# scroll-tech/scroll-prover

Measured on AMD Instinct MI355X. Metric: BN254 MSM G1-adds/sec at k=26, higher is better.
Workload: dtype u32 (9x29-bit limbs of 254-bit Montgomery integers; v_mad_u64_u32); 1 GPU; BN254 G1 Pippenger MSM, 2^26 uniform random scalars x synthetic SRS points, inputs resident in HBM; point-range shards over 1 GPU(s), RCCL all-gather of 96-B partials; log_n=26, window_bits=22, windows=12, parallelism=point-range x1, one rank per GPU, srs_window_tables=True

## Files before the change

### scroll-prover_amd/csrc/lib_msm.hip

```cpp
#define ZK_FRSCAN_DEVICE_ONLY 1
#include "msm.hpp"
#define ZK_G2_DEVICE_ONLY 1
#include "msm_g2.hpp"
#include "msm_seg.hpp"
#include "lib_common.hpp"

namespace mi355 {

static_assert(sizeof(fe_t) == 32 && sizeof(g1_affine_t) == 64 && sizeof(g1_jac_t) == 96, "ABI element sizes");
static_assert(sizeof(g1_xyzz_t) == 128 && sizeof(g1_xyzz29_t) == 144, "device record sizes (workspace layout, 16-byte vector accesses)");

int msm_tu_init_device() {
  HIPCHK(hipFuncSetAttribute((const void *)k_sort_l1_scatter_split<24>, hipFuncAttributeMaxDynamicSharedMemorySize, 160 * 1024));
  HIPCHK(hipFuncSetAttribute((const void *)k_sort_l1_scatter_split<16>, hipFuncAttributeMaxDynamicSharedMemorySize, 160 * 1024));
  HIPCHK(hipFuncSetAttribute((const void *)k_sort_l1_scatter_split<8>, hipFuncAttributeMaxDynamicSharedMemorySize, 160 * 1024));
  HIPCHK(hipFuncSetAttribute((const void *)k_sort_l2_scatter_split<16>, hipFuncAttributeMaxDynamicSharedMemorySize, 160 * 1024));
  HIPCHK(hipFuncSetAttribute((const void *)k_sort_l2_scatter_split<8>, hipFuncAttributeMaxDynamicSharedMemorySize, 160 * 1024));
  return MI355_OK;
}

double msm_cost(uint64_t n, int c, bool shared) { const double W = (MSM_SCALAR_BITS + c - 1) / c, nb = (double)(1ull << (c - 1)); return 1.18 * W * (double)n + 8.2 * nb * (shared ? 1.0 : W) + (shared ? 0.0 : 3.0e7); }

int choose_c(uint64_t n) {
  if (t_opts.force_c) return t_opts.force_c;
// ... 80 lines not shown
  int32_t *lv_ids; rec_t *lv_recs;
  CHK(ws.get("segfix_ids", cap * 4, lv_ids)); CHK(ws.get("segfix_recs", cap * sizeof(rec_t), lv_recs));
  const int32_t *cur_ids = part_id; const rec_t *cur_recs = part; size_t used = 0;
  while (N > 64) {
    const uint32_t waves = ceil_div(N, 64);
    hipLaunchKernelGGL(k_msm_segfix<G>, dim3(ceil_div(N, 256)), dim3(256), 0, s, cur_ids, cur_recs, N, buckets, lv_ids + used, lv_recs + used, 0);
    cur_ids = lv_ids + used; cur_recs = lv_recs + used; used += (size_t)2 * waves; N = 2 * waves;
  }
  hipLaunchKernelGGL(k_msm_segfix<G>, dim3(1), dim3(64), 0, s, cur_ids, cur_recs, N, buckets, (int32_t *)nullptr, (rec_t *)nullptr, 1);
  return MI355_OK;
}

template <class G> int msm_reduce_tail(const MsmShape &sh, uint32_t M, const typename G::rec_t *buckets, typename G::out_t *out_dev, bool normalise, hipStream_t s, const Roles &ws) {
  using rec_t = typename G::rec_t;
  const uint32_t nb = 1u << (sh.c - 1), wpp = sh.shared ? 1 : sh.W, sets = M * wpp;
  uint32_t chunk = 64; while (chunk > nb) chunk >>= 1;
  while (chunk > g.reduce_min_chunk && (uint64_t)(nb / chunk) * sets < g.reduce_chains) chunk >>= 1;
  const uint32_t chunks_per_set = nb / chunk, nchunks = chunks_per_set * sets;
  rec_t *chunk_out, *tree_a, *tree_b, *window_sums;
  CHK(ws.get("chunk_out", (size_t)nchunks * sizeof(rec_t), chunk_out));
  { const size_t lvl = (size_t)ceil_div(chunks_per_set, 64 * TREE_PER_THREAD) * sets + 1;
    CHK(ws.get("tree_a", lvl * sizeof(rec_t), tree_a)); CHK(ws.get("tree_b", lvl * sizeof(rec_t), tree_b)); }
  CHK(ws.get("window_sums", (size_t)sets * sizeof(rec_t), window_sums));
  with_lanes<G>(nchunks <= g.tail_coop_max && (g.tail_coop_mask & 2u), [&](auto q) {
    constexpr int Q = decltype(q)::value;
    hipLaunchKernelGGL((k_msm_bucket_reduce<G, Q>), dim3(ceil_div((uint64_t)nchunks * Q, 128)), dim3(128), 0, s, buckets, chunk_out, nb, sets, chunk);
  });
  const rec_t *cur = chunk_out; uint32_t cnt = chunks_per_set; rec_t *bufs[2] = {tree_a, tree_b}; int which = 0;
  while (true) {
    const bool coop = G::QUAD && (uint64_t)cnt * sets <= g.tail_coop_max && (g.tail_coop_mask & 4u);
    const uint32_t outn = ceil_div(cnt, (coop ? 64u : 256u) * TREE_PER_THREAD);
    rec_t *dst = outn == 1 ? window_sums : bufs[which];
    with_lanes<G>(coop, [&](auto q) { hipLaunchKernelGGL((k_msm_tree_sum<G, decltype(q)::value>), dim3(outn, sets), dim3(256), 0, s, cur, cnt, dst, outn); });
    if (outn == 1) break;
    cur = dst; cnt = outn; which ^= 1;
  }
  with_lanes<G>(g.tail_coop_max && (g.tail_coop_mask & 8u), [&](auto q) {
    hipLaunchKernelGGL((k_msm_final<G, decltype(q)::value>), dim3(M), dim3(64), 0, s, (const rec_t *)window_sums, wpp, sh.shared ? 0u : sh.c, out_dev, normalise ? 1 : 0);
  });
  HIPCHK(hipGetLastError());
  return MI355_OK;
}

int msm_sort_stage(const PolyPtrs &inl, const fe_t *const *polys_dev, uint32_t M, uint64_t n, const MsmShape &sh, const MsmPlan &P, uint32_t *offsets, uint32_t *sorted,
                   hipStream_t s, bool g2 = false) {
  const bool shared = sh.shared;
  const uint64_t emax = sh.emax;
  const uint32_t nbuckets = (uint32_t)sh.nbuckets;
  SortPlan S; S.n = P.n; S.windows = M * P.windows; S.wpp = P.windows; S.nb = P.nb;
  S.fb = sh.fb; S.cb_bits = sh.cb_bits;
  S.shared = shared ? 1 : 0; S.nshift = log2_ceil(n);
  S.regions = sh.regions;
  S.t1 = g.sort_t1;
  if (g.sort_split == 1 && S.t1 == 16384 && (1u << S.cb_bits) <= 1024 && emax >= (1ull << 24)) S.t1 = 24576;
  S.t2 = g.sort_t2 ? g.sort_t2 : (emax >= (1ull << 27) && S.fb <= 11 ? 16384 : 8192);
  const uint32_t tiles1 = ceil_div(n, S.t1), l2_tiles_max = ceil_div(emax, S.t2) + S.regions + 8;
  const uint32_t vwindows = M * P.windows;

  uint32_t *enc, *hist, *cursor, *scan_sums, *coarse_hist, *coarse_off, *coarse_cursor, *tile_start;
  CHK(ws_get("msm.digits", emax * 4, (void **)&enc));
  uint32_t *pairs_lo = nullptr; uint16_t *pairs_hi = nullptr;
  CHK(ws_get("msm.pairs_lo", emax * 4 + 64, (void **)&pairs_lo)); CHK(ws_get("msm.pairs_hi", emax * 2 + 64, (void **)&pairs_hi));
  CHK(ws_get("msm.hist", ((size_t)nbuckets + 1) * 4, (void **)&hist));
  CHK(ws_get("msm.cursor", ((size_t)nbuckets + 1) * 4, (void **)&cursor));
  CHK(ws_get("msm.coarse_hist", ((size_t)S.regions + 1) * 4, (void **)&coarse_hist));
  CHK(ws_get("msm.coarse_off", ((size_t)S.regions + 1) * 4, (void **)&coarse_off));
  CHK(ws_get("msm.coarse_cursor", ((size_t)S.regions + 1) * 4, (void **)&coarse_cursor));
  CHK(ws_get("msm.tile_start", ((size_t)S.regions + 1) * 4, (void **)&tile_start));
  const uint32_t scan_n = nbuckets + 1, scan_blocks = ceil_div(scan_n, SCAN_BLOCK * SCAN_ITEMS);
  const uint32_t cscan_n = S.regions + 1, cscan_blocks = ceil_div(cscan_n, SCAN_BLOCK * SCAN_ITEMS);
  CHK(ws_get("msm.scan_sums", (size_t)(scan_blocks + cscan_blocks) * 4, (void **)&scan_sums));
  const int grid_stream = g.prop.multiProcessorCount * 8;
  {
    Scope sc(g2 ? "msm_g2_digits" : "msm_digits", s);
    HIPCHK(hipMemsetAsync(coarse_hist, 0, ((size_t)S.regions + 1) * 4, s));
    const dim3 dgrid(grid_stream / M > 0 ? grid_stream / M : 1, M);
    if (g2) hipLaunchKernelGGL(k_msm_digits<false>, dgrid, dim3(256), (size_t)S.regions * 4, s, inl, polys_dev, enc, P, coarse_hist, S.fb, S.cb_bits, S.shared);
    else hipLaunchKernelGGL(k_msm_digits<true>, dgrid, dim3(256), (size_t)S.regions * 4, s, inl, polys_dev, enc, P, coarse_hist, S.fb, S.cb_bits, S.shared);
  }
  {
    Scope sc(g2 ? "msm_g2_sort" : "msm_sort", s);
    HIPCHK(hipMemsetAsync(hist, 0, ((size_t)nbuckets + 1) * 4, s));
    hipLaunchKernelGGL(k_scan_partial, dim3(cscan_blocks), dim3(SCAN_BLOCK), 0, s, coarse_hist, scan_sums + scan_blocks, cscan_n);
    hipLaunchKernelGGL(k_scan_block_sums, dim3(1), dim3(SCAN_BLOCK), 0, s, scan_sums + scan_blocks, cscan_blocks);
    hipLaunchKernelGGL(k_scan_final, dim3(cscan_blocks), dim3(SCAN_BLOCK), 0, s, coarse_hist, scan_sums + scan_blocks, coarse_off, coarse_cursor, cscan_n);
    {
      Scope s1(g2 ? "g2_sort_l1" : "sort_l1", s);
      const uint32_t CBp = ((1u << S.cb_bits) + 1) & ~1u;
      const size_t lds1 = (size_t)(3 * CBp + 32 + SORT_SPLIT_TMAX) * 4 + (size_t)S.t1 * 6;
      if (S.t1 == 24576) hipLaunchKernelGGL(k_sort_l1_scatter_split<24>, dim3(tiles1 * vwindows), dim3(1024), lds1, s, enc, coarse_cursor, pairs_lo, pairs_hi, S);
      else if (S.t1 == 16384) hipLaunchKernelGGL(k_sort_l1_scatter_split<16>, dim3(tiles1 * vwindows), dim3(1024), lds1, s, enc, coarse_cursor, pairs_lo, pairs_hi, S);
      else hipLaunchKernelGGL(k_sort_l1_scatter_split<8>, dim3(tiles1 * vwindows), dim3(1024), lds1, s, enc, coarse_cursor, pairs_lo, pairs_hi, S);
    }
    hipLaunchKernelGGL(k_sort_tile_prefix, dim3(1), dim3(SCAN_BLOCK), 0, s, coarse_off, tile_start, S);
    { Scope s2(g2 ? "g2_sort_hist" : "sort_hist", s);
    hipLaunchKernelGGL(k_sort_l2_hist_split, dim3(l2_tiles_max), dim3(256), 0, s, (const uint16_t *)pairs_hi, coarse_off, tile_start, hist, S); }
    hipLaunchKernelGGL(k_scan_partial, dim3(scan_blocks), dim3(SCAN_BLOCK), 0, s, hist, scan_sums, scan_n);
    hipLaunchKernelGGL(k_scan_block_sums, dim3(1), dim3(SCAN_BLOCK), 0, s, scan_sums, scan_blocks);
    hipLaunchKernelGGL(k_scan_final, dim3(scan_blocks), dim3(SCAN_BLOCK), 0, s, hist, scan_sums, offsets, cursor, scan_n);
    {
      Scope s3(g2 ? "g2_sort_l2" : "sort_l2", s);
      const size_t lds2 = (size_t)(3 * (1u << S.fb) + 32) * 4 + (size_t)S.t2 * 6;
      if (S.t2 == 8192) hipLaunchKernelGGL(k_sort_l2_scatter_split<8>, dim3(l2_tiles_max), dim3(1024), lds2, s, (const uint32_t *)pairs_lo, (const uint16_t *)pairs_hi, coarse_off, tile_start, cursor, sorted, S);
      else hipLaunchKernelGGL(k_sort_l2_scatter_split<16>, dim3(l2_tiles_max), dim3(1024), lds2, s, (const uint32_t *)pairs_lo, (const uint16_t *)pairs_hi, coarse_off, tile_start, cursor, sorted, S);
    }
  }
  return MI355_OK;
}

struct MsmStreams { hipStream_t a, b, c; };

int msm_enqueue(const g1_affine_t *bases, const PolyPtrs &inl, const fe_t *const *polys_dev, uint32_t M, uint64_t n, g1_jac_t *out_dev, const PreTable *pre, MsmSlot &slot,
                const MsmStreams &st, bool normalise, const MsmShape *forced = nullptr, uint32_t set_index = 0, uint32_t set_count = 1, bool skip_tail = false) {
  const bool piped = st.a != st.b;
  const Roles ws{G1Ops::ROLE, slot.id ? "#" + std::to_string(slot.id) : std::string()};
  MsmShape sh; CHK(msm_shape(n, M, pre, sh, forced));
  const bool shared = sh.shared;
  if (shared) bases = pre->table;
  const uint64_t emax = sh.emax;
  const AccPlan ap = msm_acc_plan(emax);
  const MsmPlan P = msm_plan(sh, n, M, ap.seg);
  const bool segfix = g.fixup_mode == 1 || (g.fixup_mode == 2 && (uint32_t)sh.nbuckets >= (1u << 19) && (uint64_t)P.seg * sh.nbuckets >= emax);
  const uint32_t seg_arg = msm_seg_arg(P.seg, segfix ? g.seg_fill_segfix : g.seg_fill);
  const uint32_t nbuckets = (uint32_t)sh.nbuckets;
  const uint32_t acc_blocks = ap.blocks, tn = ap.tn;
  uint32_t *offsets, *sorted;
  g1_xyzz29_t *buckets, *part; int32_t *part_id;
  CHK(ws.get("offsets", ((size_t)nbuckets + 1) * 4, offsets));
  CHK(ws.get("sorted", emax * 4, sorted));
  CHK(ws.get("buckets", (size_t)nbuckets * set_count * sizeof(g1_xyzz29_t), buckets));
  buckets += (size_t)nbuckets * set_index;
  CHK(ws.get("part", (size_t)tn * 2 * sizeof(g1_xyzz29_t), part));
  CHK(ws.get("part_id", (size_t)tn * 2 * 4, part_id));
  const uint32_t big_cap = tn / g.fixup_serial_max + 2;
  uint32_t *big_list; CHK(ws.get("big_list", ((size_t)big_cap * 3 + 1) * 4, big_list));
  uint32_t *big_count = big_list + (size_t)big_cap * 3;
  const uint32_t huge_cap = tn / FIXUP_HUGE_MIN + 2;
  uint32_t *huge_list, *huge_count; g1_xyzz29_t *huge_part;
  CHK(ws.get("huge_list", ((size_t)huge_cap * 3 + 1) * 4, huge_list)); huge_count = huge_list + (size_t)huge_cap * 3;
  CHK(ws.get("huge_part", (size_t)huge_cap * FIXUP_SLICES * sizeof(g1_xyzz29_t), huge_part));

  {
    hipStream_t s = st.a;
    if (piped && slot.used) { HIPCHK(hipStreamWaitEvent(s, slot.acc_done, 0)); HIPCHK(hipStreamWaitEvent(s, slot.red_done, 0)); }
    CHK(msm_sort_stage(inl, polys_dev, M, n, sh, P, offsets, sorted, s));
    if (piped) { HIPCHK(hipEventRecord(slot.sorted, s)); HIPCHK(hipStreamWaitEvent(st.b, slot.sorted, 0)); }
  }
  {
    hipStream_t s = st.b;
    if (piped && slot.used) HIPCHK(hipStreamWaitEvent(s, slot.red_done, 0));
    {
      Scope sc("msm_accumulate", s);
      HIPCHK(hipMemsetAsync(buckets, 0, (size_t)nbuckets * sizeof(g1_xyzz29_t), s));
      hipLaunchKernelGGL(k_msm_accumulate, dim3(acc_blocks), dim3(256), 0, s, bases, sorted, offsets, nbuckets, buckets, part, part_id, seg_arg, log2_ceil(n), shared ? pre->row_stride : (uint64_t)0);
    }
    if (piped) { HIPCHK(hipEventRecord(slot.acc_done, s)); HIPCHK(hipStreamWaitEvent(st.c, slot.acc_done, 0)); }
  }
  {
    hipStream_t s = st.c;
    Scope sc("msm_reduce", s);
    HIPCHK(hipMemsetAsync(big_count, 0, 4, s));
    HIPCHK(hipMemsetAsync(huge_count, 0, 4, s));
    if (segfix) CHK(msm_segfix_levels<G1Ops>(part_id, part, tn, buckets, s, ws));
    else {
      auto fixup = [&](auto kernel, uint64_t threads) {
        hipLaunchKernelGGL(kernel, dim3(ceil_div(threads, 256)), dim3(256), 0, s, offsets, nbuckets, buckets, part, part_id, seg_arg, tn, big_list, big_count, big_cap, huge_list, huge_count, huge_cap, g.fixup_serial_max, g.fixup_huge_min);
      };
      if ((uint64_t)nbuckets * 4 <= g.tail_coop_max && (g.tail_coop_mask & 1u)) fixup(k_msm_fixup<4, 4>, (uint64_t)nbuckets * 16);
      else if (nbuckets <= (1u << g.fixup_lanes_max_log)) fixup(k_msm_fixup<4, 1>, (uint64_t)nbuckets * 4);
      else fixup(k_msm_fixup<1, 1>, nbuckets);
      hipLaunchKernelGGL(k_msm_fixup_big, dim3(big_cap), dim3(256), 0, s, buckets, part, part_id, big_list, big_count);
      hipLaunchKernelGGL(k_msm_fixup_huge, dim3(huge_cap * FIXUP_SLICES), dim3(256), 0, s, part, part_id, huge_list, huge_count, huge_part, huge_cap);
      hipLaunchKernelGGL(k_msm_fixup_huge_fold, dim3(huge_cap), dim3(64), 0, s, buckets, huge_list, huge_count, (const g1_xyzz29_t *)huge_part);
    }
    if (!skip_tail) CHK(msm_reduce_tail<G1Ops>(sh, M, buckets, out_dev, normalise, s, ws));
  }
  if (piped) HIPCHK(hipEventRecord(slot.red_done, st.c));
  slot.used = true;
  HIPCHK(hipGetLastError());
  g.last_c = (int)P.c; g.last_w = (int)P.windows; g.last_entries += emax; g.last_shared = shared;
  return MI355_OK;
}

uint32_t msm_chunks_for(uint32_t M, uint64_t n) {
  if (g.msm_chunks <= 1 || M != 1 || n < (1ull << g.msm_chunk_min_log)) return 1;
  uint32_t k = g.msm_chunks;
  while (k > 1 && n / k < ((1ull << g.msm_chunk_min_log) >> 2)) k--;
  return k;
}

int msm_deliver(CallTrace &tr, const g1_jac_t *out_dev, uint32_t M, void *out_host, void *out_dev_user, hipStream_t s, const char *what, uint32_t count) {
  if (out_dev_user) {
    HIPCHK(hipMemcpyAsync(out_dev_user, out_dev, (size_t)M * sizeof(g1_jac_t), hipMemcpyDeviceToDevice, s));
    if (g.profiling) resolve_spans();
    tr.done(" (device result)");
    return MI355_OK;
  }
  HIPCHK(hipMemcpyAsync(out_host, out_dev, (size_t)M * sizeof(g1_jac_t), hipMemcpyDeviceToHost, s));
  HIPCHK(hipStreamSynchronize(s));
  resolve_spans();
  { char buf[64]; snprintf(buf, sizeof buf, " %s=%u c=%d W=%d", what, count, g.last_c, g.last_w); tr.done(buf); }
  return MI355_OK;
}

int msm_batch_impl(const g1_affine_t *bases, const fe_t *const *polys_host, uint32_t M, uint64_t n, void *out_host, const PreTable *pre, void *out_dev_user = nullptr, bool accumulate_plan = false) {
  if (M == 0) return MI355_OK;
  if (n == 0) {
    if (out_dev_user) { HIPCHK(hipMemsetAsync(out_dev_user, 0, (size_t)M * sizeof(g1_jac_t), g.stream)); return MI355_OK; }
    memset(out_host, 0, (size_t)M * sizeof(g1_jac_t)); return MI355_OK;
  }
  if (n >= (1ull << 31)) return fail(MI355_EBADARG, "msm: n must be < 2^31");
  if (M > 1 && msm_batch_must_split<G1Ops>(n, M, pre)) {
    const uint32_t h = M / 2;
    CHK(msm_batch_impl(bases, polys_host, h, n, out_host, pre, out_dev_user, accumulate_plan));
    return msm_batch_impl(bases, polys_host + h, M - h, n, out_host ? (char *)out_host + (size_t)h * sizeof(g1_jac_t) : nullptr, pre,
                          out_dev_user ? (char *)out_dev_user + (size_t)h * sizeof(g1_jac_t) : nullptr, true);
  }
  const uint32_t K = msm_chunks_for(M, n);
  if (!accumulate_plan) { g.last_entries = 0; g.last_host_slices = 1; }
  CallTrace tr("msm_g1", (uint64_t)M * n, 96.0);
  g1_jac_t *out_dev; const fe_t **polys_dev = nullptr;
  CHK(ws_get("msm.out", (size_t)(K + 1) * M * sizeof(g1_jac_t), (void **)&out_dev));
  hipStream_t s = g.stream;
  Scope total("msm_total", s);
  PolyPtrs inl{};
  if (K == 1) {
    CHK(msm_stage_polys(polys_host, M, Roles{G1Ops::ROLE, ""}, s, inl, polys_dev));
    MsmStreams st{s, s, s};
    CHK(msm_enqueue(bases, inl, polys_dev, M, n, out_dev, pre, g.msm_slot[0], st, t_opts.normalise));
  } else {
    std::vector<uint64_t> lo(K + 1);
    for (uint32_t k = 0; k <= K; k++) lo[k] = n * k / K;
    HIPCHK(hipEventRecord(g.ev_fork, s));
    HIPCHK(hipStreamWaitEvent(g.aux_stream[0], g.ev_fork, 0)); HIPCHK(hipStreamWaitEvent(g.aux_stream[1], g.ev_fork, 0));
    MsmStreams st{g.aux_stream[0], s, g.aux_stream[1]};
    for (uint32_t k = 0; k < K; k++) {
      PreTable pk; const PreTable *pp = pre_advance(pre, lo[k], pk);
      inl.p[0] = polys_host[0] + lo[k];
      CHK(msm_enqueue(bases + lo[k], inl, nullptr, M, lo[k + 1] - lo[k], out_dev + (size_t)(k + 1) * M, pp, g.msm_slot[k & 1], st, false));
    }
    HIPCHK(hipStreamWaitEvent(s, g.msm_slot[0].red_done, 0)); HIPCHK(hipStreamWaitEvent(s, g.msm_slot[1].red_done, 0));
    HIPCHK(hipEventRecord(g.ev_fork, st.a)); HIPCHK(hipStreamWaitEvent(s, g.ev_fork, 0));
    hipLaunchKernelGGL(k_g1_sum_strided, dim3(M), dim3(64), 0, s, out_dev + M, K, M, out_dev, t_opts.normalise ? 1 : 0);
  }
  HIPCHK(hipGetLastError());
  total.close();
  g.msm_slot[0].used = g.msm_slot[1].used = false;
  g.last_chunks = (int)K;
  return msm_deliver(tr, out_dev, M, out_host, out_dev_user, s, "batch", M);
}

int msm_host_single(const g1_affine_t *bases, const fe_t *const *polys_host, uint32_t M, uint64_t n, void *out_host, const PreTable *pre, void *out_dev_user = nullptr) {
  fe_t *sc; CHK(ws_get("io.scalars", (size_t)M * n * sizeof(fe_t), (void **)&sc));
  hipStream_t s = g.stream;
  std::vector<uint64_t> cut;
  if (M == 1 && n >= (1ull << g.host_slice_min_log) && g.host_chunks > 1) {
    double w = 1.0, tot = 0; std::vector<double> ws;
    const double first = 1.0 / 16.0;
    for (double rem = 1.0; rem > 1e-9 && ws.size() + 1 < g.host_chunks;) { const double take = std::min(rem, first * w); ws.push_back(take); rem -= take; w *= 1.7; tot += take; }
    if (tot < 1.0 - 1e-9) ws.push_back(1.0 - tot);
    cut.push_back(0); double acc = 0;
    const uint64_t align = n >= (1ull << 20) ? ~1023ull : ~0ull;
    for (size_t i = 0; i + 1 < ws.size(); i++) { acc += ws[i]; const uint64_t c = std::min<uint64_t>(n, (uint64_t)(acc * (double)n) & align); if (c > cut.back() && c < n) cut.push_back(c); }
    cut.push_back(n);
  }
  uint32_t K = cut.empty() ? 1 : (uint32_t)cut.size() - 1;
  uint64_t biggest = 0; for (uint32_t k = 0; k < K && !cut.empty(); k++) biggest = std::max(biggest, cut[k + 1] - cut[k]);
  MsmShape shape;
  if (K > 1 && (msm_shape(biggest, 1, pre, shape) != MI355_OK || shape.nbuckets * K * sizeof(g1_xyzz29_t) > (8ull << 30))) K = 1;
  if (K <= 1) {
    std::vector<const fe_t *> ptrs(M);
    for (uint32_t m = 0; m < M; m++) { ptrs[m] = sc + (size_t)m * n; HIPCHK(hipMemcpyAsync(sc + (size_t)m * n, polys_host[m], n * sizeof(fe_t), hipMemcpyHostToDevice, s)); }
    return msm_batch_impl(bases, ptrs.data(), M, n, out_host, pre, out_dev_user);
  }
  g.last_entries = 0;
  CallTrace tr("msm_g1_host", n, 96.0);
  g1_jac_t *out_dev; CHK(ws_get("msm.out", 2 * sizeof(g1_jac_t), (void **)&out_dev));
  Scope total("msm_total", s);
  HIPCHK(hipEventRecord(g.ev_fork, s)); HIPCHK(hipStreamWaitEvent(g.copy_stream, g.ev_fork, 0));
  PolyPtrs inl{};
  MsmStreams st{s, s, s};
  for (uint32_t k = 0; k < K; k++) {
    const uint64_t lo = cut[k], hi = cut[k + 1];
    HIPCHK(hipMemcpyAsync(sc + lo, polys_host[0] + lo, (hi - lo) * sizeof(fe_t), hipMemcpyHostToDevice, g.copy_stream));
    HIPCHK(hipEventRecord(g.ev_copy[k & 3], g.copy_stream));
    HIPCHK(hipStreamWaitEvent(s, g.ev_copy[k & 3], 0));
    PreTable pk; const PreTable *pp = pre_advance(pre, lo, pk);
    inl.p[0] = sc + lo;
    CHK(msm_enqueue(bases + lo, inl, nullptr, 1, hi - lo, out_dev, pp, g.msm_slot[0], st, t_opts.normalise, &shape, k, K, true));
  }
  g.msm_slot[0].used = false;
  g1_xyzz29_t *buckets; CHK(ws_get("msm.buckets", (size_t)shape.nbuckets * K * sizeof(g1_xyzz29_t), (void **)&buckets));
  {
    Scope sc2("msm_reduce", s);
    hipLaunchKernelGGL(k_msm_bucket_fold, dim3(ceil_div(shape.nbuckets, 256)), dim3(256), 0, s, buckets, (uint32_t)shape.nbuckets, K);
    CHK(msm_reduce_tail<G1Ops>(shape, 1, buckets, out_dev, t_opts.normalise, s, Roles{G1Ops::ROLE, ""}));
  }
  total.close();
  g.last_chunks = (int)K; g.last_host_slices = (int)K;
  return msm_deliver(tr, out_dev, 1, out_host, out_dev_user, s, "host slices", K);
}

static int msm_g2_impl(const g2_affine_t *bases, const fe_t *const *polys, uint32_t M, uint64_t n, void *out_host, bool accumulate_plan = false) {
  if (M == 0) return MI355_OK;
  if (n == 0) { memset(out_host, 0, (size_t)M * sizeof(g2_affine_t)); return MI355_OK; }
  if (n >= (1ull << 31)) return fail(MI355_EBADARG, "msm_g2: n must be < 2^31");
// ... 618 lines not shown
```

### scroll-prover_amd/csrc/msm.hpp

```cpp
#pragma once
#include "fp_asm.hpp"
#include "g1_29.hpp"
#include "frscan.hpp"

namespace zk {

#if defined(__HIPCC__)

struct MsmPlan {
  uint32_t n;
  uint32_t c;
  uint32_t windows;
  uint32_t nb;
  uint32_t seg;
  uint32_t batch;
};

__device__ __forceinline__ g1_affine_t load_affine(const g1_affine_t *p) {
  g1_affine_t r; r.x = g_load(&p->x); r.y = g_load(&p->y); return r;
}
__device__ __forceinline__ g1_affine_t load_affine_nt(const g1_affine_t *p) {
  const uint32_t *q = reinterpret_cast<const uint32_t *>(p); g1_affine_t r;
#pragma unroll
  for (int i = 0; i < 8; i++) { r.x.l[i] = __builtin_nontemporal_load(q + i); r.y.l[i] = __builtin_nontemporal_load(q + 8 + i); }
// ... 213 lines not shown
__device__ __forceinline__ void tile_bin_publish(uint32_t *gbase, const uint32_t *lstart, const uint32_t (&gb)[4], uint32_t nbins) {
  const uint32_t bpt = (nbins + 1023) >> 10, b0 = threadIdx.x * bpt;
  for (uint32_t k = 0; k < 4; k++) if (k < bpt && b0 + k < nbins) gbase[b0 + k] = gb[k] - lstart[b0 + k];
}
template <int EPT> __global__ void __launch_bounds__(1024) k_sort_l1_scatter_split(const uint32_t *__restrict__ enc, uint32_t *__restrict__ coarse_cursor, uint32_t *__restrict__ pairs_lo,
                                                                                    uint16_t *__restrict__ pairs_hi, SortPlan S) {
  extern __shared__ uint32_t sm[];
  const uint32_t CB = 1u << S.cb_bits, CBp = (CB + 1) & ~1u, fmask = (1u << S.fb) - 1;
  const uint32_t spare = 16u - S.fb, rmask = (1u << spare) - 1, tcount = (CB + rmask) >> spare;
  uint32_t *h = sm, *lstart = sm + CBp, *gbase = sm + 2 * CBp, *scratch32 = sm + 3 * CBp, *T = sm + 3 * CBp + 32;
  uint32_t *stage_lo = T + SORT_SPLIT_TMAX;
  uint16_t *stage_hi = reinterpret_cast<uint16_t *>(stage_lo + 1024 * EPT);
  const uint32_t tiles1 = (S.n + S.t1 - 1) / S.t1;
  const uint32_t w = blockIdx.x / tiles1, j = blockIdx.x - w * tiles1;
  for (uint32_t b = threadIdx.x; b < CB; b += 1024) h[b] = 0;
  __syncthreads();
  const uint32_t i0 = j * S.t1, i1 = min(S.n, i0 + S.t1);
  const uint32_t *plane = enc + (uint64_t)w * S.n;
  uint32_t e[EPT], rank[EPT];
#pragma unroll
  for (int k = 0; k < EPT; k++) {
    const uint32_t i = i0 + k * 1024 + threadIdx.x;
    e[k] = i < i1 ? plane[i] : 0;
  }
  asm volatile("s_waitcnt vmcnt(0)" ::: "memory");
#pragma unroll
  for (int k = 0; k < EPT; k++) if (e[k]) rank[k] = atomicAdd(&h[((e[k] & 0x7fffffffu) - 1) >> S.fb], 1u);
  __syncthreads();
  const uint32_t m_poly = w / S.wpp, w_in = w - m_poly * S.wpp;
  uint32_t gb[4];
  const uint32_t total = tile_bin_offsets(h, lstart, gb, CB, coarse_cursor + (S.shared ? m_poly * CB : w * CB), scratch32);
  const uint32_t idx_base = S.shared ? w_in << S.nshift : 0;
  __syncthreads();
  for (uint32_t k = threadIdx.x; k < tcount; k += 1024) T[k] = lstart[k << spare];
#pragma unroll
  for (int k = 0; k < EPT; k++) if (e[k]) {
    const uint32_t bucket = (e[k] & 0x7fffffffu) - 1, i = i0 + k * 1024 + threadIdx.x, bin = bucket >> S.fb, pos = lstart[bin] + rank[k];
    stage_lo[pos] = (idx_base + i) | (e[k] & 0x80000000u);
    stage_hi[pos] = (uint16_t)((bucket & fmask) | ((bin & rmask) << S.fb));
  }
  tile_bin_publish(gbase, lstart, gb, CB);
  __syncthreads();
  uint32_t k = 0;
  for (uint32_t sidx = threadIdx.x; sidx < total; sidx += 1024) {
    const uint32_t key = stage_hi[sidx];
    while (k + 1 < tcount && T[k + 1] <= sidx) k++;
    const uint32_t bin = (k << spare) | (key >> S.fb), pos = gbase[bin] + sidx;
    pairs_lo[pos] = stage_lo[sidx]; pairs_hi[pos] = (uint16_t)(key & fmask);
  }
}
__global__ void __launch_bounds__(SCAN_BLOCK) k_sort_tile_prefix(const uint32_t *__restrict__ coarse_off, uint32_t *__restrict__ tile_start, SortPlan S) {
  __shared__ uint32_t lds[32];
  __shared__ uint32_t running;
  if (threadIdx.x == 0) running = 0;
  __syncthreads();
  for (uint32_t base = 0; base < S.regions; base += SCAN_BLOCK) {
    const uint32_t r = base + threadIdx.x;
    const uint32_t v = r < S.regions ? (coarse_off[r + 1] - coarse_off[r] + S.t2 - 1) / S.t2 : 0;
    uint32_t total; const uint32_t ex = block_exclusive_scan(v, lds, total);
    const uint32_t run = running;
    if (r < S.regions) tile_start[r] = run + ex;
    __syncthreads();
    if (threadIdx.x == 0) running = run + total;
    __syncthreads();
  }
  if (threadIdx.x == 0) tile_start[S.regions] = running;
}
__device__ __forceinline__ bool sort_l2_tile(const uint32_t *__restrict__ coarse_off, const uint32_t *__restrict__ tile_start, const SortPlan &S, uint32_t &region, uint32_t &s, uint32_t &e) {
  const uint32_t total = tile_start[S.regions], per_xcd = (total + 7) >> 3, q = blockIdx.x >> 3;
  const uint32_t tile = (blockIdx.x & 7) * per_xcd + q;
  if (q >= per_xcd || tile >= total) return false;
  uint32_t lo = 0, hi = S.regions;
  while (hi - lo > 1) { const uint32_t mid = (lo + hi) >> 1; if (tile_start[mid] <= tile) lo = mid; else hi = mid; }
  region = lo;
  s = coarse_off[lo] + (tile - tile_start[lo]) * S.t2;
  e = min(coarse_off[lo + 1], s + S.t2);
  return true;
}
__global__ void __launch_bounds__(256) k_sort_l2_hist_split(const uint16_t *__restrict__ pairs_hi, const uint32_t *__restrict__ coarse_off, const uint32_t *__restrict__ tile_start,
                                                            uint32_t *__restrict__ hist, SortPlan S) {
  __shared__ uint32_t h[SORT_MAX_BINS];
  uint32_t region, s, e;
  if (!sort_l2_tile(coarse_off, tile_start, S, region, s, e)) return;
  const uint32_t FB = 1u << S.fb;
  for (uint32_t b = threadIdx.x; b < FB; b += blockDim.x) h[b] = 0;
  __syncthreads();
  const uint32_t a0 = min(e, (s + 7u) & ~7u), a1 = a0 + ((e - a0) & ~7u);
  for (uint32_t p = s + threadIdx.x; p < a0; p += blockDim.x) atomicAdd(&h[pairs_hi[p]], 1u);
  for (uint32_t q = a0 + 8u * threadIdx.x; q < a1; q += 8u * blockDim.x) {
    const uint4 v = *reinterpret_cast<const uint4 *>(pairs_hi + q);
    atomicAdd(&h[v.x & 0xffffu], 1u); atomicAdd(&h[v.x >> 16], 1u); atomicAdd(&h[v.y & 0xffffu], 1u); atomicAdd(&h[v.y >> 16], 1u);
    atomicAdd(&h[v.z & 0xffffu], 1u); atomicAdd(&h[v.z >> 16], 1u); atomicAdd(&h[v.w & 0xffffu], 1u); atomicAdd(&h[v.w >> 16], 1u);
  }
  for (uint32_t p = a1 + threadIdx.x; p < e; p += blockDim.x) atomicAdd(&h[pairs_hi[p]], 1u);
  __syncthreads();
  for (uint32_t b = threadIdx.x; b < FB; b += blockDim.x) if (h[b]) atomicAdd(&hist[(region << S.fb) + b], h[b]);
}
template <int EPT> __global__ void __launch_bounds__(1024) k_sort_l2_scatter_split(const uint32_t *__restrict__ pairs_lo, const uint16_t *__restrict__ pairs_hi, const uint32_t *__restrict__ coarse_off,
                                                                                    const uint32_t *__restrict__ tile_start, uint32_t *__restrict__ cursor, uint32_t *__restrict__ sorted, SortPlan S) {
  extern __shared__ uint32_t sm[];
  const uint32_t FB = 1u << S.fb;
  uint32_t *h = sm, *lstart = sm + FB, *gbase = sm + 2 * FB, *scratch32 = sm + 3 * FB, *stage = sm + 3 * FB + 32;
  uint32_t region, s, e;
  if (!sort_l2_tile(coarse_off, tile_start, S, region, s, e)) return;
  for (uint32_t b = threadIdx.x; b < FB; b += 1024) h[b] = 0;
  __syncthreads();
  uint32_t idx[EPT], fine[EPT], rank[EPT];
#pragma unroll
  for (int k = 0; k < EPT; k++) {
    const uint32_t p = s + k * 1024 + threadIdx.x;
    fine[k] = 0xffffffffu;
    if (p < e) { idx[k] = pairs_lo[p]; fine[k] = pairs_hi[p]; }
  }
  asm volatile("s_waitcnt vmcnt(0)" ::: "memory");
#pragma unroll
  for (int k = 0; k < EPT; k++) if (fine[k] != 0xffffffffu) rank[k] = atomicAdd(&h[fine[k]], 1u);
  __syncthreads();
  uint32_t gb[4];
  const uint32_t total = tile_bin_offsets(h, lstart, gb, FB, cursor + (region << S.fb), scratch32);
  __syncthreads();
  uint16_t *stage_bin = reinterpret_cast<uint16_t *>(stage + 1024 * EPT);
#pragma unroll
  for (int k = 0; k < EPT; k++) if (fine[k] != 0xffffffffu) { const uint32_t pos = lstart[fine[k]] + rank[k]; stage[pos] = idx[k]; stage_bin[pos] = (uint16_t)fine[k]; }
  tile_bin_publish(gbase, lstart, gb, FB);
  __syncthreads();
  for (uint32_t sidx = threadIdx.x; sidx < total; sidx += 1024) {
    const uint32_t b = stage_bin[sidx];
    sorted[gbase[b] + sidx] = stage[sidx];
  }
}

__device__ __forceinline__ uint32_t msm_seg_eff(uint32_t total, uint32_t threads, uint32_t seg_arg) {
  const uint32_t seg_max = seg_arg & 0x1fffu, seg_min = (seg_arg >> 13) & 0x1fffu, fill_pct = (seg_arg >> 26) * 2;
  const uint64_t target = ((uint64_t)threads * (fill_pct > 100u ? 100u : fill_pct) + 99) / 100;
  uint32_t sg = (uint32_t)(((uint64_t)total + target - 1) / (target ? target : 1));
  sg = sg < seg_min ? seg_min : sg;
  return sg > seg_max ? seg_max : sg;
}
template <class G, class B> __device__ __forceinline__ void msm_segment_walk(const B &bases, const uint32_t *__restrict__ sorted, const uint32_t *__restrict__ offsets, uint32_t nbuckets,
                                                                              typename G::rec_t *__restrict__ bucket_sums, typename G::rec_t *__restrict__ part, int32_t *__restrict__ part_id, uint32_t seg_arg,
                                                                              uint32_t t, uint32_t threads) {
  const uint32_t total = offsets[nbuckets];
  const uint32_t seg = msm_seg_eff(total, threads, seg_arg);
  const uint64_t start64 = (uint64_t)t * seg;
  if (start64 >= total) { part_id[2 * t] = -1; part_id[2 * t + 1] = -1; return; }
  const uint32_t start = (uint32_t)start64, end = (uint32_t)min((uint64_t)total, start64 + seg);
  uint32_t lo = 0, hi = nbuckets;
  while (hi - lo > 1) { const uint32_t mid = (lo + hi) >> 1; if (offsets[mid] <= start) lo = mid; else hi = mid; }
  uint32_t b = lo, b_start = offsets[b], b_end = offsets[b + 1];
  int32_t id_first = -1, id_last = -1;
  typename G::rec_t acc = G::identity();
  uint32_t ent = sorted[start];
  uint32_t ent_next = start + 1 < end ? sorted[start + 1] : 0;
  typename B::base_t p = bases.load(ent);
  for (uint32_t pos = start; pos < end; pos++) {
    typename B::base_t p_next = p;
    if (pos + 1 < end) { ent_next = sorted[pos + 1]; p_next = bases.load(ent_next); }
    if (pos >= b_end) {
      if (b_start >= start) G::store(&bucket_sums[b], acc);
      else { G::store(&part[2 * (uint64_t)t], acc); id_first = (int32_t)b; }
      acc = G::identity();
      b++; b_start = b_end; b_end = offsets[b + 1];
      if (pos >= b_end) {
        uint32_t l2 = b, h2 = nbuckets;
        while (h2 - l2 > 1) { const uint32_t mid = (l2 + h2) >> 1; if (offsets[mid] <= pos) l2 = mid; else h2 = mid; }
        b = l2; b_start = offsets[b]; b_end = offsets[b + 1];
      }
    }
    bases.madd(acc, p, (ent >> 31) != 0);
    ent = ent_next; p = p_next;
  }
  if (b_start >= start && b_end <= end) G::store(&bucket_sums[b], acc);
  else if (b_start < start) { G::store(&part[2 * (uint64_t)t], acc); id_first = (int32_t)b; }
  else { G::store(&part[2 * (uint64_t)t + 1], acc); id_last = (int32_t)b; }
  part_id[2 * t] = id_first; part_id[2 * t + 1] = id_last;
}
struct G1Bases {
  using base_t = g1_affine_t;
  const g1_affine_t *__restrict__ bases; uint32_t nshift; uint64_t row_stride;
  __device__ __forceinline__ const g1_affine_t *base_of(uint32_t e) const {
    const uint32_t gi = e & 0x7fffffffu;
    if (row_stride == 0) return &bases[gi];
    const uint32_t w = gi >> nshift;
    return &bases[(uint64_t)w * row_stride + (gi & ((1u << nshift) - 1))];
  }
  __device__ __forceinline__ g1_affine_t load(uint32_t e) const { return load_affine(base_of(e)); }
  __device__ __forceinline__ void madd(g1_xyzz29_t &acc, const g1_affine_t &p, bool neg) const { g1_xyzz29_madd(acc, p, neg); }
};
struct G1AccOps : G1Ops {
  static __device__ __forceinline__ void store(rec_t *p, rec_t v) { g1_xyzz29_negx_to_plain(v); store_xyzz29(p, v); }
};
__global__ void __launch_bounds__(256) k_msm_accumulate(const g1_affine_t *__restrict__ bases, const uint32_t *__restrict__ sorted, const uint32_t *__restrict__ offsets,
                                                        uint32_t nbuckets, g1_xyzz29_t *__restrict__ bucket_sums, g1_xyzz29_t *__restrict__ part, int32_t *__restrict__ part_id, uint32_t seg_arg,
                                                        uint32_t nshift, uint64_t row_stride) {
  msm_segment_walk<G1AccOps>(G1Bases{bases, nshift, row_stride}, sorted, offsets, nbuckets, bucket_sums, part, part_id, seg_arg, blockIdx.x * blockDim.x + threadIdx.x, gridDim.x * blockDim.x);
}

constexpr uint32_t FIXUP_SERIAL_MAX = 32, FIXUP_HUGE_MIN = 2048, FIXUP_SLICES = 64;
template <int Q = 1> __device__ __forceinline__ void fixup_take29(g1_xyzz29_t &acc, const g1_xyzz29_t *__restrict__ part, const int32_t *__restrict__ part_id, uint32_t t, uint32_t b) {
  if (part_id[2 * t] == (int32_t)b) g1_vadd<Q>(acc, load_xyzz29(&part[2 * (uint64_t)t]));
  else if (part_id[2 * t + 1] == (int32_t)b) g1_vadd<Q>(acc, load_xyzz29(&part[2 * (uint64_t)t + 1]));
}
template <uint32_t FIXUP_LANES, int Q = 1> __global__ void __launch_bounds__(256) k_msm_fixup(const uint32_t *__restrict__ offsets, uint32_t nbuckets, g1_xyzz29_t *__restrict__ bucket_sums,
                                                   const g1_xyzz29_t *__restrict__ part, const int32_t *__restrict__ part_id, uint32_t seg_arg, uint32_t acc_threads,
                                                   uint32_t *__restrict__ big_list, uint32_t *__restrict__ big_count, uint32_t big_cap,
                                                   uint32_t *__restrict__ huge_list, uint32_t *__restrict__ huge_count, uint32_t huge_cap, uint32_t serial_max, uint32_t huge_min) {
  const uint32_t gid = (blockIdx.x * blockDim.x + threadIdx.x) / Q, b = gid / FIXUP_LANES, sub = gid % FIXUP_LANES;
  const bool lead = (threadIdx.x & (Q - 1)) == 0;
  const uint32_t seg = msm_seg_eff(offsets[nbuckets], acc_threads, seg_arg);
  g1_xyzz29_t acc = g1_xyzz29_identity();
  bool mine = false;
  if (b < nbuckets) {
    const uint32_t s = offsets[b], e = offsets[b + 1];
    if (e != s) {
      const uint32_t t0 = s / seg, t1 = (e - 1) / seg;
      if (t0 != t1) {
        if (t1 - t0 > serial_max) {
          if (sub == 0 && lead) {
            if (huge_cap && t1 - t0 >= huge_min) {
              const uint32_t idx = atomicAdd(huge_count, 1u);
              if (idx < huge_cap) { huge_list[3 * idx] = b; huge_list[3 * idx + 1] = t0; huge_list[3 * idx + 2] = t1; }
            } else {
              const uint32_t idx = atomicAdd(big_count, 1u);
              if (idx < big_cap) { big_list[3 * idx] = b; big_list[3 * idx + 1] = t0; big_list[3 * idx + 2] = t1; }
            }
          }
        } else {
          mine = true;
          for (uint32_t t = t0 + sub; t <= t1; t += FIXUP_LANES) fixup_take29<Q>(acc, part, part_id, t, b);
        }
      }
    }
  }
  if (FIXUP_LANES > 1) { const g1_xyzz29_t other = shfl_xor_xyzz29(acc, 1 * Q); g1_vadd<Q>(acc, other); }
  if (FIXUP_LANES > 2) { const g1_xyzz29_t other = shfl_xor_xyzz29(acc, 2 * Q); g1_vadd<Q>(acc, other); }
  static_assert(FIXUP_LANES == 1 || FIXUP_LANES == 2 || FIXUP_LANES == 4, "two shuffle steps");
  if (mine && sub == 0 && lead) store_xyzz29(&bucket_sums[b], acc);
}
__global__ void __launch_bounds__(256) k_msm_fixup_big(g1_xyzz29_t *__restrict__ bucket_sums, const g1_xyzz29_t *__restrict__ part, const int32_t *__restrict__ part_id,
                                                       const uint32_t *__restrict__ big_list, const uint32_t *__restrict__ big_count) {
  __shared__ g1_xyzz29_t lds29[4];
  if (blockIdx.x >= *big_count) return;
  const uint32_t b = big_list[3 * blockIdx.x], t0 = big_list[3 * blockIdx.x + 1], t1 = big_list[3 * blockIdx.x + 2];
  g1_xyzz29_t acc = g1_xyzz29_identity();
  for (uint32_t t = t0 + threadIdx.x; t <= t1; t += blockDim.x) fixup_take29(acc, part, part_id, t, b);
  for (uint32_t o = 32; o >= 1; o >>= 1) { const g1_xyzz29_t other = shfl_down_xyzz29(acc, o); g1_xyzz29_add(acc, other); }
  if ((threadIdx.x & 63) == 0) lds29[threadIdx.x >> 6] = acc;
  __syncthreads();
  if (threadIdx.x == 0) { for (uint32_t k = 1; k < (blockDim.x >> 6); k++) g1_xyzz29_add(acc, lds29[k]); store_xyzz29(&bucket_sums[b], acc); }
}
__device__ __forceinline__ uint32_t fixup_huge_slices(uint32_t span) { const uint32_t s = span >> 11; return s < 1u ? 1u : (s > FIXUP_SLICES ? FIXUP_SLICES : s); }
__global__ void __launch_bounds__(256) k_msm_fixup_huge(const g1_xyzz29_t *__restrict__ part, const int32_t *__restrict__ part_id, const uint32_t *__restrict__ huge_list,
                                                        const uint32_t *__restrict__ huge_count, g1_xyzz29_t *__restrict__ huge_part, uint32_t huge_cap) {
  __shared__ g1_xyzz29_t lds29[4];
  const uint32_t count = min(*huge_count, huge_cap);
  if (count == 0) return;
  const uint32_t sl = blockIdx.x / count, idx = blockIdx.x - sl * count;
  if (sl >= FIXUP_SLICES) return;
  const uint32_t b = huge_list[3 * idx], t0 = huge_list[3 * idx + 1], t1 = huge_list[3 * idx + 2], span = t1 - t0 + 1;
  const uint32_t nsl = fixup_huge_slices(span);
  if (sl >= nsl) return;
  const uint32_t lo = t0 + (uint32_t)((uint64_t)span * sl / nsl), hi = t0 + (uint32_t)((uint64_t)span * (sl + 1) / nsl);
  g1_xyzz29_t acc = g1_xyzz29_identity();
  for (uint32_t t = lo + threadIdx.x; t < hi; t += blockDim.x) fixup_take29(acc, part, part_id, t, b);
  for (uint32_t o = 32; o >= 1; o >>= 1) { const g1_xyzz29_t other = shfl_down_xyzz29(acc, o); g1_xyzz29_add(acc, other); }
  if ((threadIdx.x & 63) == 0) lds29[threadIdx.x >> 6] = acc;
  __syncthreads();
  if (threadIdx.x == 0) { for (uint32_t k = 1; k < (blockDim.x >> 6); k++) g1_xyzz29_add(acc, lds29[k]); store_xyzz29(&huge_part[(uint64_t)idx * FIXUP_SLICES + sl], acc); }
}
__global__ void __launch_bounds__(64) k_msm_fixup_huge_fold(g1_xyzz29_t *__restrict__ bucket_sums, const uint32_t *__restrict__ huge_list, const uint32_t *__restrict__ huge_count,
                                                            const g1_xyzz29_t *__restrict__ huge_part) {
  const uint32_t idx = blockIdx.x;
  if (idx >= *huge_count) return;
  const uint32_t nsl = fixup_huge_slices(huge_list[3 * idx + 2] - huge_list[3 * idx + 1] + 1);
  g1_xyzz29_t acc = threadIdx.x < nsl ? load_xyzz29(&huge_part[(uint64_t)idx * FIXUP_SLICES + threadIdx.x]) : g1_xyzz29_identity();
  for (uint32_t o = FIXUP_SLICES / 2; o >= 1; o >>= 1) { const g1_xyzz29_t other = shfl_down_xyzz29(acc, o); g1_xyzz29_add(acc, other); }
  if (threadIdx.x == 0) store_xyzz29(&bucket_sums[huge_list[3 * idx]], acc);
}

template <class G> __global__ void __launch_bounds__(256) k_msm_segfix(const int32_t *__restrict__ ids, const typename G::rec_t *__restrict__ recs, uint32_t n, typename G::rec_t *__restrict__ bucket_sums,
                                                    int32_t *__restrict__ ids_out, typename G::rec_t *__restrict__ recs_out, int last_level) {
  using rec_t = typename G::rec_t;
  const uint32_t j = blockIdx.x * blockDim.x + threadIdx.x, lane = threadIdx.x & 63, wave = j >> 6;
  if (wave >= ((n + 63) >> 6)) return;
  const int32_t key0 = j < n ? ids[j] : -1;
  rec_t val = key0 >= 0 ? G::load(&recs[j]) : G::identity();
  int32_t key = key0;
  for (uint32_t o = 1; o < 64; o <<= 1) { const int32_t kk = __shfl_up(key, o); if (lane >= o && key < 0) key = kk; }
  for (uint32_t o = 1; o < 64; o <<= 1) {
    const int32_t k2 = __shfl_down(key, o);
    const bool take = lane + o < 64 && key >= 0 && k2 == key;
    if (__ballot(take) == 0) continue;
    const rec_t other = G::shfl_down(val, o);
    if (take) G::template add<1>(val, other);
  }
  const int32_t kprev = __shfl_up(key, 1);
  const bool head = key >= 0 && (lane == 0 || kprev != key);
  const uint64_t valid = __ballot(key >= 0);
  const uint32_t first_lane = valid ? (uint32_t)__ffsll((unsigned long long)valid) - 1 : 64u;
  const int32_t key_last = __shfl(key, 63), key_first = __shfl(key, first_lane < 64u ? (int)first_lane : 0);
  const bool is_first = head && lane == first_lane, is_last = head && key == key_last;
  if (last_level) { if (head) G::store(&bucket_sums[key], val); return; }
  if (head && !is_first && !is_last) G::store(&bucket_sums[key], val);
  if (is_first) { ids_out[2 * wave] = key; G::store(&recs_out[2 * (uint64_t)wave], val); }
  if (is_last && !is_first) { ids_out[2 * wave + 1] = key; G::store(&recs_out[2 * (uint64_t)wave + 1], val); }
  if (lane == 0) {
    if (first_lane == 64u) { ids_out[2 * wave] = -1; ids_out[2 * wave + 1] = -1; }
    else if (key_first == key_last) ids_out[2 * wave + 1] = -1;
  }
}

__global__ void __launch_bounds__(256) k_msm_bucket_fold(g1_xyzz29_t *__restrict__ buckets, uint32_t nbuckets, uint32_t sets) {
  const uint32_t b = blockIdx.x * blockDim.x + threadIdx.x;
  if (b >= nbuckets) return;
  g1_xyzz29_t acc = load_xyzz29(&buckets[b]);
  for (uint32_t k = 1; k < sets; k++) g1_xyzz29_add(acc, load_xyzz29(&buckets[(uint64_t)k * nbuckets + b]));
  store_xyzz29(&buckets[b], acc);
}

template <class G, int Q> __global__ void __launch_bounds__(128) k_msm_bucket_reduce(const typename G::rec_t *__restrict__ bucket_sums, typename G::rec_t *__restrict__ chunk_out, uint32_t nb, uint32_t sets, uint32_t chunk) {
  using rec_t = typename G::rec_t;
  const uint32_t chunks_per_set = nb / chunk;
  const uint32_t gi = (blockIdx.x * blockDim.x + threadIdx.x) / Q;
  if (gi >= chunks_per_set * sets) return;
  const uint32_t w = gi / chunks_per_set, j = gi - w * chunks_per_set;
  const rec_t *B = bucket_sums + (uint64_t)w * nb + (uint64_t)j * chunk;
  rec_t run = G::identity(), T = G::identity();
  for (uint32_t i = chunk; i-- > 0;) { G::template add<Q>(run, G::load(&B[i])); G::template add<Q>(T, run); }
  if (j != 0) {
    const uint32_t k = j * chunk;
    rec_t kS = G::identity();
    for (int bit = 31 - __clz(k); bit >= 0; bit--) { kS = G::template dbl<Q>(kS); if ((k >> bit) & 1) G::template add<Q>(kS, run); }
    G::template add<Q>(T, kS);
  }
  if ((threadIdx.x & (Q - 1)) == 0) G::store(&chunk_out[gi], T);
}
constexpr uint32_t TREE_PER_THREAD = 4;
template <class G, int Q> __global__ void __launch_bounds__(256) k_msm_tree_sum(const typename G::rec_t *__restrict__ in, uint32_t in_per_set, typename G::rec_t *__restrict__ out, uint32_t out_per_set) {
  using rec_t = typename G::rec_t;
  __shared__ rec_t lds[4];
  constexpr uint32_t VT = 256 / Q;
  const uint32_t w = blockIdx.y, first = blockIdx.x * VT * TREE_PER_THREAD, vt = threadIdx.x / Q;
  const rec_t *src = in + (uint64_t)w * in_per_set;
  rec_t acc = G::identity();
  for (uint32_t k = 0; k < TREE_PER_THREAD; k++) { const uint32_t i = first + k * VT + vt; if (i < in_per_set) G::template add<Q>(acc, G::load(&src[i])); }
  for (uint32_t o = 32 / Q; o >= 1; o >>= 1) { const rec_t other = G::shfl_down(acc, o * Q); G::template add<Q>(acc, other); }
  if ((threadIdx.x & 63) == 0) lds[threadIdx.x >> 6] = acc;
  __syncthreads();
// ... 116 lines not shown
```

### scroll-prover_amd/csrc/msm_g2.hpp

```cpp
#pragma once
#include "msm.hpp"
#include "g2.hpp"

namespace zk {

#if defined(__HIPCC__)

static_assert(sizeof(g2_affine_t) == 128 && sizeof(g2_xyzz_t) == 256, "G2 record sizes (16-byte vector accesses)");

__device__ __forceinline__ g2_affine_t load_g2_affine(const g2_affine_t *p) {
  g2_affine_t r; uint32_t *w = reinterpret_cast<uint32_t *>(&r); const uint4 *q = reinterpret_cast<const uint4 *>(p);
#pragma unroll
  for (int i = 0; i < 8; i++) { const uint4 a = q[i]; w[4 * i] = a.x; w[4 * i + 1] = a.y; w[4 * i + 2] = a.z; w[4 * i + 3] = a.w; }
  return r;
}
__device__ __forceinline__ g2_xyzz_t load_g2_xyzz(const g2_xyzz_t *p) {
  g2_xyzz_t r; uint32_t *w = reinterpret_cast<uint32_t *>(&r); const uint4 *q = reinterpret_cast<const uint4 *>(p);
#pragma unroll
  for (int i = 0; i < 16; i++) { const uint4 a = q[i]; w[4 * i] = a.x; w[4 * i + 1] = a.y; w[4 * i + 2] = a.z; w[4 * i + 3] = a.w; }
  return r;
}
__device__ __forceinline__ void store_g2_xyzz(g2_xyzz_t *p, const g2_xyzz_t &v) {
  const uint32_t *w = reinterpret_cast<const uint32_t *>(&v); uint4 *q = reinterpret_cast<uint4 *>(p);
#pragma unroll
  for (int i = 0; i < 16; i++) q[i] = make_uint4(w[4 * i], w[4 * i + 1], w[4 * i + 2], w[4 * i + 3]);
}
__device__ __forceinline__ g2_xyzz_t shfl_down_g2(const g2_xyzz_t &v, uint32_t o) {
  g2_xyzz_t r; const uint32_t *s = reinterpret_cast<const uint32_t *>(&v); uint32_t *d = reinterpret_cast<uint32_t *>(&r);
#pragma unroll
  for (int i = 0; i < 64; i++) d[i] = __shfl_down(s[i], o);
  return r;
}

__global__ void __launch_bounds__(256) k_msm_g2_validate(const g2_affine_t *__restrict__ pts, uint64_t n, fe2_t b, uint32_t *__restrict__ first_bad) {
  const uint64_t stride = (uint64_t)gridDim.x * blockDim.x;
  for (uint64_t i = (uint64_t)blockIdx.x * blockDim.x + threadIdx.x; i < n; i += stride)
    if (!g2_is_on_curve_b<Fq2ps>(load_g2_affine(&pts[i]), b)) atomicMin(first_bad, (uint32_t)i);
}

struct G2Ops {
  using rec_t = g2_xyzz_t; using out_t = g2_affine_t;
  static constexpr bool QUAD = false;
  static constexpr const char *ROLE = "msm2.";
  static __device__ __forceinline__ rec_t identity() { return g2_xyzz_identity(); }
  static __device__ __forceinline__ rec_t load(const rec_t *p) { return load_g2_xyzz(p); }
  static __device__ __forceinline__ void store(rec_t *p, const rec_t &v) { store_g2_xyzz(p, v); }
  template <int Q> static __device__ __forceinline__ void add(rec_t &acc, const rec_t &o) { static_assert(Q == 1, "G2 has no quad form"); g2_xyzz_add<Fq2ps>(acc, o); }
  template <int Q> static __device__ __forceinline__ rec_t dbl(const rec_t &a) { static_assert(Q == 1, "G2 has no quad form"); return g2_xyzz_dbl<Fq2ps>(a); }
  static __device__ __forceinline__ rec_t shfl_down(const rec_t &v, uint32_t o) { return shfl_down_g2(v, o); }
  static __device__ __forceinline__ void emit(const rec_t &acc, out_t *out, int) { *out = g2_xyzz_to_affine<Fq2ps>(acc); }
};

struct G2Bases {
  using base_t = g2_affine_t;
  const g2_affine_t *__restrict__ bases;
  __device__ __forceinline__ g2_affine_t load(uint32_t e) const { return load_g2_affine(&bases[e & 0x7fffffffu]); }
  __device__ __forceinline__ void madd(g2_xyzz_t &acc, g2_affine_t p, bool neg) const {
    if (neg) p.y = Fq2ps::neg(p.y);
    g2_xyzz_madd<Fq2ps>(acc, p);
  }
};
__global__ void __launch_bounds__(256) k_msm_g2_accumulate(const g2_affine_t *__restrict__ bases, const uint32_t *__restrict__ sorted, const uint32_t *__restrict__ offsets,
                                                          uint32_t nbuckets, g2_xyzz_t *__restrict__ bucket_sums, g2_xyzz_t *__restrict__ part, int32_t *__restrict__ part_id, uint32_t seg_arg) {
  msm_segment_walk<G2Ops>(G2Bases{bases}, sorted, offsets, nbuckets, bucket_sums, part, part_id, seg_arg, blockIdx.x * blockDim.x + threadIdx.x, gridDim.x * blockDim.x);
}

#endif

}
```

Before: 12.37 billion G1-adds/s.

## Stage bucket-accumulate base loads through LDS with double-buffered direct-to-LDS prefetch

```diff
diff --git a/scroll-prover_amd/csrc/lib_msm.hip b/scroll-prover_amd/csrc/lib_msm.hip
--- a/scroll-prover_amd/csrc/lib_msm.hip
+++ b/scroll-prover_amd/csrc/lib_msm.hip
@@ -256,6 +256,7 @@
     {
       Scope sc("msm_accumulate", s);
       HIPCHK(hipMemsetAsync(buckets, 0, (size_t)nbuckets * sizeof(g1_xyzz29_t), s));
+      static_assert(MSM_ACC_STAGE_LANES == 256, "k_msm_accumulate stages one base per lane of this workgroup size");
       hipLaunchKernelGGL(k_msm_accumulate, dim3(acc_blocks), dim3(256), 0, s, bases, sorted, offsets, nbuckets, buckets, part, part_id, seg_arg, log2_ceil(n), shared ? pre->row_stride : (uint64_t)0);
     }
     if (piped) { HIPCHK(hipEventRecord(slot.acc_done, s)); HIPCHK(hipStreamWaitEvent(st.c, slot.acc_done, 0)); }
diff --git a/scroll-prover_amd/csrc/msm.hpp b/scroll-prover_amd/csrc/msm.hpp
--- a/scroll-prover_amd/csrc/msm.hpp
+++ b/scroll-prover_amd/csrc/msm.hpp
@@ -389,10 +389,19 @@
   typename G::rec_t acc = G::identity();
   uint32_t ent = sorted[start];
   uint32_t ent_next = start + 1 < end ? sorted[start + 1] : 0;
-  typename B::base_t p = bases.load(ent);
+  typename B::base_t p;
+  uint32_t slot = 0;
+  if constexpr (B::lds_prefetch) bases.prefetch(ent, 0); else p = bases.load(ent);
   for (uint32_t pos = start; pos < end; pos++) {
-    typename B::base_t p_next = p;
-    if (pos + 1 < end) { ent_next = sorted[pos + 1]; p_next = bases.load(ent_next); }
+    typename B::base_t p_next;
+    uint32_t ent_after = 0;
+    if constexpr (B::lds_prefetch) {
+      p = bases.take(slot);
+      if (pos + 1 < end) { bases.prefetch(ent_next, slot ^ 1u); if (pos + 2 < end) ent_after = sorted[pos + 2]; }
+    } else {
+      p_next = p;
+      if (pos + 1 < end) { ent_next = sorted[pos + 1]; p_next = bases.load(ent_next); }
+    }
     if (pos >= b_end) {
       if (b_start >= start) G::store(&bucket_sums[b], acc);
       else { G::store(&part[2 * (uint64_t)t], acc); id_first = (int32_t)b; }
@@ -405,16 +414,36 @@
       }
     }
     bases.madd(acc, p, (ent >> 31) != 0);
-    ent = ent_next; p = p_next;
+    if constexpr (B::lds_prefetch) { ent = ent_next; ent_next = ent_after; slot ^= 1u; }
+    else { ent = ent_next; p = p_next; }
   }
   if (b_start >= start && b_end <= end) G::store(&bucket_sums[b], acc);
   else if (b_start < start) { G::store(&part[2 * (uint64_t)t], acc); id_first = (int32_t)b; }
   else { G::store(&part[2 * (uint64_t)t + 1], acc); id_last = (int32_t)b; }
   part_id[2 * t] = id_first; part_id[2 * t + 1] = id_last;
 }
+constexpr uint32_t MSM_ACC_STAGE_LANES = 256, MSM_ACC_STAGE_BYTES = 2 * 4 * MSM_ACC_STAGE_LANES * 16;
 struct G1Bases {
   using base_t = g1_affine_t;
+  static constexpr bool lds_prefetch = true;
   const g1_affine_t *__restrict__ bases; uint32_t nshift; uint64_t row_stride;
+  uint4 *stage;
+  __device__ __forceinline__ void prefetch(uint32_t e, uint32_t slot) const {
+    const char *src = reinterpret_cast<const char *>(base_of(e));
+    uint4 *dst = stage + slot * (4 * MSM_ACC_STAGE_LANES) + (threadIdx.x & ~63u);
+#pragma unroll
+    for (uint32_t k = 0; k < 4; k++)
+      __builtin_amdgcn_global_load_lds((const __attribute__((address_space(1))) void *)(src + 16 * k), (__attribute__((address_space(3))) void *)(dst + k * MSM_ACC_STAGE_LANES), 16, 0, 0);
+  }
+  __device__ __forceinline__ g1_affine_t take(uint32_t slot) const {
+    asm volatile("s_waitcnt vmcnt(0)" ::: "memory");
+    const uint4 *src = stage + slot * (4 * MSM_ACC_STAGE_LANES) + threadIdx.x;
+    const uint4 a = src[0], b = src[MSM_ACC_STAGE_LANES], c = src[2 * MSM_ACC_STAGE_LANES], d = src[3 * MSM_ACC_STAGE_LANES];
+    g1_affine_t r;
+    r.x.l[0] = a.x; r.x.l[1] = a.y; r.x.l[2] = a.z; r.x.l[3] = a.w; r.x.l[4] = b.x; r.x.l[5] = b.y; r.x.l[6] = b.z; r.x.l[7] = b.w;
+    r.y.l[0] = c.x; r.y.l[1] = c.y; r.y.l[2] = c.z; r.y.l[3] = c.w; r.y.l[4] = d.x; r.y.l[5] = d.y; r.y.l[6] = d.z; r.y.l[7] = d.w;
+    return r;
+  }
   __device__ __forceinline__ const g1_affine_t *base_of(uint32_t e) const {
     const uint32_t gi = e & 0x7fffffffu;
     if (row_stride == 0) return &bases[gi];
@@ -430,7 +459,8 @@
 __global__ void __launch_bounds__(256) k_msm_accumulate(const g1_affine_t *__restrict__ bases, const uint32_t *__restrict__ sorted, const uint32_t *__restrict__ offsets,
                                                         uint32_t nbuckets, g1_xyzz29_t *__restrict__ bucket_sums, g1_xyzz29_t *__restrict__ part, int32_t *__restrict__ part_id, uint32_t seg_arg,
                                                         uint32_t nshift, uint64_t row_stride) {
-  msm_segment_walk<G1AccOps>(G1Bases{bases, nshift, row_stride}, sorted, offsets, nbuckets, bucket_sums, part, part_id, seg_arg, blockIdx.x * blockDim.x + threadIdx.x, gridDim.x * blockDim.x);
+  __shared__ uint4 stage[MSM_ACC_STAGE_BYTES / sizeof(uint4)];
+  msm_segment_walk<G1AccOps>(G1Bases{bases, nshift, row_stride, stage}, sorted, offsets, nbuckets, bucket_sums, part, part_id, seg_arg, blockIdx.x * blockDim.x + threadIdx.x, gridDim.x * blockDim.x);
 }
 
 constexpr uint32_t FIXUP_SERIAL_MAX = 32, FIXUP_HUGE_MIN = 2048, FIXUP_SLICES = 64;
diff --git a/scroll-prover_amd/csrc/msm_g2.hpp b/scroll-prover_amd/csrc/msm_g2.hpp
--- a/scroll-prover_amd/csrc/msm_g2.hpp
+++ b/scroll-prover_amd/csrc/msm_g2.hpp
@@ -53,6 +53,7 @@
 
 struct G2Bases {
   using base_t = g2_affine_t;
+  static constexpr bool lds_prefetch = false;
   const g2_affine_t *__restrict__ bases;
   __device__ __forceinline__ g2_affine_t load(uint32_t e) const { return load_g2_affine(&bases[e & 0x7fffffffu]); }
   __device__ __forceinline__ void madd(g2_xyzz_t &acc, g2_affine_t p, bool neg) const {
```

Result: no change. 12.44 billion G1-adds/s (median of 6 runs) (+0.6%).
